# Const-me/Whisper

Hardware: AMD Instinct MI355X
Metric: audio-seconds/sec (real-time factor), ggml-medium & large, 30s chunks @1/2/4/8 GPU (higher is better)
Workload: dtype f16

## Files before the change

### whisper_amd/binding.py

```python
from __future__ import annotations

import ctypes as C
import os
from typing import Optional, Sequence

import numpy as np

from . import ggml_format as gf

_HERE = os.path.dirname(os.path.abspath(__file__))
LIB_PATH = os.path.join(_HERE, "lib", "libwhisper_hip.so")

WH_FLAG_PARITY_PV = 1
WH_FLAG_NO_GRAPH = 2
WH_FLAG_DEBUG_CAPTURE = 4
WH_FLAG_PARITY_EXACT = 8
TUNE_GEMM_8WAVE = 16
TUNE_GEMM_4WAVE = 4
TUNE_GEMM_FAST_EPI = 1
TUNE_GEMV_ROWS4, TUNE_GEMM_BIG, TUNE_GEMV_SMALLREG, TUNE_GEMM_GL, TUNE_LN_SEPARATE_BIGM, TUNE_ATTN_XCD = 2, 8, 32, 64, 128, 256
TUNE_ATTN_DEC_G, TUNE_FUSE_CROSS_Q, TUNE_GEMM_GROUP_M, TUNE_FUSE_SELF_BLOCK, TUNE_GEMV_LN_BLOCK, TUNE_GEMV_K8 = 512, 1024, 2048, 4096, 8192, 16384
TUNE_SPLIT_STREAMS, TUNE_ATTN_ENC_F, TUNE_GEMM_WIDE_EPI, TUNE_GEMM_FRAGPF, TUNE_ATTN_ENC_2SWEEP = 32768, 65536, 131072, 262144, 524288
TUNE_GEMV_ALLROWS, TUNE_GEMV_ROWGROUPS, TUNE_SELF_MFMA, TUNE_MEL_MFMA = 1048576, 2097152, 4194304, 8388608
TUNE_DECODE_SMALL, TUNE_DECODE_PREFETCH, TUNE_ATTN_DEC_NT, TUNE_ENC_SERIAL = 16777216, 33554432, 67108864, 134217728
# ... 95 lines not shown
        L.wh_context_destroy.restype = None
        L.wh_context_set_flags.argtypes = [vp, C.c_uint32, i32]
        L.wh_context_set_audio_ctx.argtypes = [vp, i32]
        L.wh_context_memory.argtypes = [vp, C.POINTER(i64)]
        L.wh_context_synchronize.argtypes = [vp]
        L.wh_buffer_upload_async.argtypes = [vp, vp, vp, i64]
        L.wh_mel_spectrogram.argtypes = [vp, vp, i64, vp, C.POINTER(i64)]
        L.wh_encode.argtypes = [vp, vp, i32, i64, i64, vp]
        L.wh_encode_windows.argtypes = [vp, vp, i32]
        L.wh_decode.argtypes = [vp, vp, i32, i32, i32, vp, vp]
        L.wh_sample_best.argtypes = [vp, i32, i32, i32, C.POINTER(TokenDataC)]
        L.wh_beam_candidates.argtypes = [vp, i32, i32, i32, i32, C.POINTER(TokenDataC)]
        L.wh_reorder_self_cache.argtypes = [vp, i32, vp, i32]
        L.wh_debug_read.argtypes = [vp, C.c_char_p, i32, i32, vp, i64]
        L.wh_decode_greedy.argtypes = [vp, i32, vp, i32, i32, i32, i32, C.POINTER(TokenDataC)]
        L.wh_decode_window_start.argtypes = [vp, i32, vp, i32, i32, i32, i32]
        L.wh_decode_window_finish.argtypes = [vp, C.POINTER(TokenDataC)]
        L.wh_decode_window_start_ragged.argtypes = [vp, i32, vp, vp, i32, i32, i32, i32]
        L.wh_decode_window_ready.argtypes = [vp, i32, i32]
        L.wh_decode_window_continue.argtypes = [vp, i32]
        L.wh_decode_window_fetch.argtypes = [vp, i32, i32, C.POINTER(TokenDataC)]
        L.wh_mel_spectrogram_window.argtypes = [vp, vp, i64, i64, i64, i64, i32, vp]
        L.wh_mel_spectrogram_batch.argtypes = [vp, vp, i64, i64, i32, vp, i64]
        L.wh_debug_probe.argtypes = [vp, i32, i32, i32, i32, i32, i32, C.POINTER(C.c_float)]
        L.wh_profile_enable.argtypes = [vp, i32]
        L.wh_profile_read.argtypes = [vp, C.POINTER(ProfileEntryC), i32, C.POINTER(i32)]
        L.wh_op_mul_mat.argtypes = [vp, vp, vp, vp, vp, vp, i32, i32, i32]
        L.wh_op_mul_mat_gelu.argtypes = [vp, vp, vp, vp, vp, i32, i32, i32]
        L.wh_op_layer_norm.argtypes = [vp, vp, vp, vp, vp, i32, i32]
        L.wh_op_flash_attention.argtypes = [vp, vp, vp, vp, vp, i32, i32, i32]
        L.wh_op_soft_max.argtypes = [vp, vp, i32, i32]
        L.wh_op_decoder_attention.argtypes = [vp, vp, vp, vp, vp, i32, i32, i32, i32, i32, i32, i32, i32, i32]
        L.wh_op_decoder_cross_attention.argtypes = [vp, vp, vp, vp, vp, vp, C.c_float, vp, vp, vp, i32, i32, i32, i32, i32]
        L.wh_op_vocab_soft_max.argtypes = [vp, vp, vp, i32, i32]
        L.wh_op_sample_best.argtypes = [vp, vp, i32, i32, i32, i32, i32, i32, i32, i32, vp]
        L.wh_op_beam_candidates.argtypes = [vp, vp, i32, i32, i32, i32, i32, i32, i32, i32, i32, vp]
        L.wh_op_reorder_self_cache.argtypes = [vp, vp, vp, vp, vp, vp, vp, i32, i32, i32, i32, i32, i32]
        L.wh_lang_detect.argtypes = [vp, i32, vp, vp]
        L.wh_model_lang_count.argtypes = [vp]
        L.wh_op_lang_probs.argtypes = [vp, vp, i32, i32, i32, i32, vp, vp]
        _lib = L
    return _lib


def check(rc: int):
    if rc != 0:
        raise WhisperHipError("libwhisper_hip rc=%d: %s" % (rc, lib().wh_last_error().decode(errors="replace")))


def set_option(name: str, value: int):
    check(lib().wh_debug_set_option(name.encode(), int(value)))


OPTION_DEFAULTS = {"dec_tile": 0, "dec_depth": 0, "dec_wide_rows": 1, "dec_deep_rows": 0, "vocab_decrows": 0, "enc_chunk": 128, "self_fuse_max_rows": 32, "self_nq": 0, "self_wave_min_rows": 32, "enc_exp": 5, "exact_enc_layers": -1, "exact_alt_order": 0, "gemm_mf16": 1, "dec_lds": 1, "dec_lds_ks": 2, "dec_split": 1, "cross_mfma": 1, "vocab_lds": 1, "beam_regs": 1, "reorder_group": 1, "gemm_big_min_rows": 8192}


def get_option(name: str) -> int:
    v = C.c_int(0)
    check(lib().wh_debug_get_option(name.encode(), C.byref(v)))
    return v.value


def get_option_default(name: str) -> int:
    return OPTION_DEFAULTS[name]


def device_count() -> int:
    return lib().wh_device_count()


def device_info(device: int = 0):
    name = C.create_string_buffer(256)
    mem = C.c_uint64()
    cus = C.c_int()
    check(lib().wh_device_info(device, name, 256, C.byref(mem), C.byref(cus)))
    return dict(name=name.value.decode(), total_mem=mem.value, compute_units=cus.value)


def _hp_c(hp: gf.HParams) -> HParamsC:
    return HParamsC(*hp.as_list())


def arena_bytes(hp: gf.HParams) -> int:
    n = lib().wh_model_arena_bytes(C.byref(_hp_c(hp)))
    if n < 0:
        check(-1)
    return int(n)


class HipModel:

    def __init__(self, hp: gf.HParams, arena_ptr: int = 0, already_filled: bool = False, keepalive=None):
        self.hp = hp
        self.handle = C.c_void_p()
        self._keepalive = keepalive
        check(lib().wh_model_create(C.byref(_hp_c(hp)), C.c_void_p(arena_ptr) if arena_ptr else None, int(already_filled),
                                    C.byref(self.handle)))

    @classmethod
    def from_ggml(cls, model: gf.GgmlModel, arena_ptr: int = 0, keepalive=None) -> "HipModel":
        m = cls(model.hparams, arena_ptr, False, keepalive)
        L = lib()
        filt = np.ascontiguousarray(model.filters, np.float32)
        check(L.wh_model_set_filters(m.handle, filt.shape[0], filt.shape[1], filt.ctypes.data_as(C.c_void_p)))
        for name, a in model.tensors.items():
            a = np.ascontiguousarray(a)
            ne = (C.c_int32 * a.ndim)(*reversed(a.shape))
# ... 327 lines not shown
```

### whisper_amd/build.py

```python
from __future__ import annotations

import os
import subprocess
import sys
import time
from concurrent.futures import ThreadPoolExecutor

HERE = os.path.dirname(os.path.abspath(__file__))
ROOT = os.path.dirname(HERE)
CSRC = os.path.join(HERE, "csrc")
HOST = os.path.join(HERE, "host")
LIB_DIR = os.path.join(HERE, "lib")
HIP_LIB = os.path.join(LIB_DIR, "libwhisper_hip.so")
HOST_LIB = os.path.join(LIB_DIR, "libWhisper.so")
CLI_BIN = os.path.join(LIB_DIR, "whisper-main")

RUNTIME_SOURCES = ["options.hip", "model.hip", "comm.hip", "context.hip", "encode.hip", "exact_graphs.hip", "decode.hip", "beam.hip", "ops_debug.hip"]
HIP_SOURCES = ["gemm.hip", "decode1.hip", "attn_enc.hip", "attn_dec.hip", "elementwise.hip", "mel.hip", "exact.hip"] + RUNTIME_SOURCES
EXTRA_FLAGS = {"exact.hip": ["-ffp-contract=off"]}
HIPCC = os.environ.get("HIPCC", "/opt/rocm/bin/hipcc")
ARCH = "gfx950"


def _newer(target: str, deps) -> bool:
    if not os.path.exists(target):
        return True
    t = os.path.getmtime(target)
    return any(os.path.getmtime(d) > t for d in deps)


def _run(cmd):
    print("+", " ".join(cmd), flush=True)
    r = subprocess.run(cmd, stdout=subprocess.PIPE, stderr=subprocess.STDOUT, text=True)
    if r.returncode != 0:
        sys.stderr.write(r.stdout)
        raise RuntimeError("build step failed: " + " ".join(cmd))
    return r.stdout


def build_hip(force: bool = False) -> str:
    os.makedirs(LIB_DIR, exist_ok=True)
    objs = []
    headers = [os.path.join(CSRC, h) for h in ("common.h", "kernels.h", "epilogue.h", "exact_ops.h")] + [os.path.join(ROOT, "include", "whisper_hip.h")]
    obj_dir = os.path.join(LIB_DIR, "obj")
    os.makedirs(obj_dir, exist_ok=True)
    stale = []
    for s in HIP_SOURCES:
        src = os.path.join(CSRC, s)
        obj = os.path.join(obj_dir, s.replace(".hip", ".o"))
        deps = [src] + headers + ([os.path.join(CSRC, "runtime.h")] if s in RUNTIME_SOURCES else [])
        if force or _newer(obj, deps):
            probes = ["-DWH_PROBES"] if os.environ.get("WH_PROBES", "") not in ("", "0") else []
            stale.append([HIPCC, "--offload-arch=" + ARCH, "-O3", "-std=c++17", "-fPIC", "-fvisibility=hidden", "-Wno-unused-result"] + probes + EXTRA_FLAGS.get(s, []) +
                         ["-I" + os.path.join(ROOT, "include"), "-c", src, "-o", obj])
        objs.append(obj)
    with ThreadPoolExecutor(max_workers=max(1, min(16, int(os.environ.get("MAX_JOBS", "0") or 0) or os.cpu_count() or 1))) as pool:
        list(pool.map(_run, stale))
    if force or _newer(HIP_LIB, objs):
        _run([HIPCC, "--offload-arch=" + ARCH, "-shared", "-fPIC", "-o", HIP_LIB] + objs + ["-ldl"])
    return HIP_LIB


def build_host(force: bool = False):
    if not os.path.isdir(HOST):
        return None
    srcs = sorted(os.path.join(HOST, f) for f in os.listdir(HOST) if f.endswith(".cpp"))
    if not srcs:
        return None
    hdrs = [os.path.join(HOST, f) for f in os.listdir(HOST) if f.endswith(".h")]
    hdrs += [os.path.join(ROOT, "include", f) for f in os.listdir(os.path.join(ROOT, "include"))]
    if force or _newer(HOST_LIB, srcs + hdrs + [HIP_LIB]):
        _run(["g++", "-std=c++17", "-O2", "-fPIC", "-shared", "-fvisibility=hidden", "-I" + os.path.join(ROOT, "include"), "-I" + HOST,
# ... 77 lines not shown
```

### whisper_amd/csrc/attn_enc.hip

```cpp
#include "kernels.h"
#include <type_traits>

namespace wh
{
	namespace
	{
		constexpr int AQ = 64;
		constexpr int AWAVES = 8;
		constexpr int QSTRIDE = 72;
		constexpr int OSTRIDE = 65;
		constexpr int ATT_LDS_BYTES = AQ * QSTRIDE * 2 + 2 * AWAVES * AQ * 4 + AWAVES * AQ * 8 + 4 * AQ * OSTRIDE * 4;

		template<int KT>
		__global__ void __launch_bounds__( 512, 2 ) attentionEnc( const f16* __restrict__ q, const f16* __restrict__ k,
			const f16* __restrict__ vT, f16* __restrict__ out, int heads, int T, int Tpad, int nQ, int xcdRemap )
		{
			extern __shared__ __attribute__( ( aligned( 16 ) ) ) unsigned char smem[];
			f16* const ldsQ = (f16*)smem;
			float* const redMax = (float*)( smem + AQ * QSTRIDE * 2 );
			float* const redInv = redMax + AWAVES * AQ;
			double* const redSum = (double*)( redInv + AWAVES * AQ );
			float* const obuf = (float*)( redSum + AWAVES * AQ );

			const int tid = threadIdx.x;
// ... 624 lines not shown
							P[ r >> 3 ][ ( r & 7 ) + 1 ] = ldsTab[ mag[ 1 ] ];
						}
						else
						{
							typedef float f2 __attribute__( ( ext_vector_type( 2 ) ) );
							constexpr float L2E = 1.44269504088896340736f;
							const h2 hp = __builtin_convertvector( f2{ S[ r ] - mx, S[ r + 1 ] - mx }, h2 );
							const f2 e = { __builtin_amdgcn_exp2f( __builtin_fmaf( (float)hp[ 0 ], L2E, 0.0f ) ), __builtin_amdgcn_exp2f( __builtin_fmaf( (float)hp[ 1 ], L2E, 0.0f ) ) };
							const h2 eh = __builtin_convertvector( e, h2 );
							P[ r >> 3 ][ r & 7 ] = eh[ 0 ];
							P[ r >> 3 ][ ( r & 7 ) + 1 ] = eh[ 1 ];
						}
					}
					sum += (double)sumP( P );
	#pragma unroll
					for( int half = 0; half < 2; half++ )
					{
						const int kb = st * 2 + half;
	#pragma unroll
						for( int ddt = 0; ddt < 2; ddt++ )
						{
							const f16x8 vf = *(const f16x8*)( vt + ( ( kb * 2 + ddt ) * 64 + lane ) * 8 );
							O[ ddt ] = __builtin_amdgcn_mfma_f32_32x32x16_f16( vf, P[ half ], O[ ddt ], 0, 0, 0 );
						}
					}
				}
			}
			sum += __shfl_xor( sum, 32, 64 );
			const float invSum = (float)( 1.0 / sum );
	#pragma unroll
			for( int a = 0; a < 2; a++ )
	#pragma unroll
				for( int r = 0; r < 16; r++ ) O[ a ][ r ] *= invSum;
			if( qRow < T )
			{
				const int b = bh / heads, h = bh - b * heads;
				f16* const o = out + ( (long long)b * T + qRow ) * ( heads * HEAD_DIM ) + h * HEAD_DIM;
	#pragma unroll
				for( int ddt = 0; ddt < 2; ddt++ )
	#pragma unroll
					for( int g4 = 0; g4 < 4; g4++ )
					{
						f16x4 pk;
	#pragma unroll
						for( int e = 0; e < 4; e++ ) pk[ e ] = (f16)O[ ddt ][ 4 * g4 + e ];
						*(f16x4*)( o + ddt * 32 + 8 * g4 + 4 * hi ) = pk;
					}
			}
		}

		constexpr int W_NBUF = 4;
		constexpr int W_LDS_BYTES = 2 * W_NBUF * F_TILE * 2;
		constexpr float W_LAZY = 4.0f;
		template<int NG, bool ONLINE, bool NOARG = false>
		__global__ void __launch_bounds__( 1024 / NG, NG == 1 ? 4 : 2 ) attentionEncW( const f16* __restrict__ q, const f16* __restrict__ k,
			const f16* __restrict__ vT, f16* __restrict__ out, int heads, int T, int Tpad, int nQ, int xcdRemap )
		{
			extern __shared__ __attribute__( ( aligned( 16 ) ) ) unsigned char smemW[];
			f16* const ldsK = (f16*)smemW;
			f16* const ldsV = ldsK + W_NBUF * F_TILE;
			typedef __attribute__( ( address_space( 3 ) ) ) void* LdsPtr;
			typedef const __attribute__( ( address_space( 1 ) ) ) void* GlobalPtr;
			typedef _Float16 h2 __attribute__( ( ext_vector_type( 2 ) ) );
			typedef float f2 __attribute__( ( ext_vector_type( 2 ) ) );
			constexpr float L2E = 1.44269504088896340736f;

			const int tid = threadIdx.x;
			const int lane = tid & 63;
			const int wave = tid >> 6;
			const int hi = lane >> 5;
			const int c = lane & 31;
			int bh, qb;
			{
				const int L = blockIdx.x;
				if( xcdRemap )
				{
					const int kIdx = L >> 3;
					bh = ( L & 7 ) + 8 * ( kIdx / nQ );
					qb = kIdx % nQ;
				}
				else
				{
					bh = L / nQ;
					qb = L - bh * nQ;
				}
			}
			const f16* const Q = q + (long long)bh * T * HEAD_DIM;
			const f16* const K = k + (long long)bh * T * HEAD_DIM;
			const f16* const VT = vT + (long long)bh * HEAD_DIM * Tpad;
			const int nTiles = ( T + FK - 1 ) / FK;
			int qRow[ NG ];
			f16x8 qf[ NG ][ 4 ];
	#pragma unroll
			for( int g = 0; g < NG; g++ )
			{
				qRow[ g ] = qb * TQ + ( wave * NG + g ) * 32 + c;
				const int qr = qRow[ g ] < T ? qRow[ g ] : T - 1;
	#pragma unroll
				for( int kk = 0; kk < 4; kk++ )
				{
					qf[ g ][ kk ] = *(const f16x8*)( Q + (long long)qr * HEAD_DIM + kk * 16 + hi * 8 );
	#pragma unroll
					for( int j = 0; j < 8; j++ ) qf[ g ][ kk ][ j ] = qf[ g ][ kk ][ j ] * (f16)0.125f;
				}
			}
			auto issueK = [ & ]( int t, int buf )
			{
	#pragma unroll
				for( int i = 0; i < NG; i++ )
				{
					const int row = ( wave * NG + i ) * 8 + ( lane >> 3 );
					const int cl = ( lane & 7 ) ^ ( ( row >> 1 ) & 7 );
					int key = t * FK + row;
					key = key < T ? key : T - 1;
					__builtin_amdgcn_global_load_lds( (GlobalPtr)( K + (long long)key * HEAD_DIM + cl * 8 ),
						(LdsPtr)( ldsK + buf * F_TILE + ( wave * NG + i ) * 512 ), 16, 0, 0 );
				}
			};
			auto issueV = [ & ]( int t, int buf )
			{
	#pragma unroll
				for( int i = 0; i < NG; i++ )
					__builtin_amdgcn_global_load_lds( (GlobalPtr)( VT + (long long)t * F_TILE + ( wave * NG + i ) * 512 + lane * 8 ),
						(LdsPtr)( ldsV + buf * F_TILE + ( wave * NG + i ) * 512 ), 16, 0, 0 );
			};
			auto waitTile = [ & ]( int t, auto per )
			{
				constexpr int P = decltype( per )::value;
				const int younger = min( W_NBUF - 2, nTiles - 1 - t );
				if( younger >= 2 )
				{
					if constexpr( P == 2 ) asm volatile( "s_waitcnt vmcnt(4)" ::: "memory" );
					else asm volatile( "s_waitcnt vmcnt(8)" ::: "memory" );
				}
				else if( younger == 1 )
				{
					if constexpr( P == 2 ) asm volatile( "s_waitcnt vmcnt(2)" ::: "memory" );
					else asm volatile( "s_waitcnt vmcnt(4)" ::: "memory" );
				}
				else asm volatile( "s_waitcnt vmcnt(0)" ::: "memory" );
			};
			static_assert( W_NBUF == 4 && NG == 2, "waitTile counts two younger tiles of 2 or 4 load instructions" );
			const f32x16 zero16 = { 0, 0, 0, 0, 0, 0, 0, 0, 0, 0, 0, 0, 0, 0, 0, 0 };
			auto scores = [ & ]( const f16* kt, int st, int t, auto last, f32x16 ( &S )[ NG ] )
			{
				const int row = st * 32 + c;
				const int sw = ( row >> 1 ) & 7;
	#pragma unroll
				for( int kk = 0; kk < 4; kk++ )
				{
					const f16x8 kf = *(const f16x8*)( kt + row * HEAD_DIM + ( ( ( kk * 2 + hi ) ^ sw ) << 3 ) );
	#pragma unroll
					for( int g = 0; g < NG; g++ ) S[ g ] = __builtin_amdgcn_mfma_f32_32x32x16_f16( kf, qf[ g ][ kk ], kk == 0 ? zero16 : S[ g ], 0, 0, 0 );
				}
				if constexpr( decltype( last )::value )
				{
					const int limit = T - ( t * FK + st * 32 + 4 * hi );
	#pragma unroll
					for( int r = 0; r < 16; r++ )
					{
						const bool in = ( r & 3 ) + 8 * ( r >> 2 ) < limit;
	#pragma unroll
						for( int g = 0; g < NG; g++ ) S[ g ][ r ] = in ? S[ g ][ r ] : -3.0e38f;
					}
				}
			};
			auto sumP = [ & ]( const f16x8 ( &P )[ 2 ] ) -> float
			{
				const h2 ones = { (f16)1.0f, (f16)1.0f };
				float part = 0.0f;
	#pragma unroll
				for( int h = 0; h < 2; h++ )
	#pragma unroll
					for( int j = 0; j < 8; j += 2 )
						part = __builtin_amdgcn_fdot2( h2{ P[ h ][ j ], P[ h ][ j + 1 ] }, ones, part, false );
				return part;
			};
			auto expTile = [ & ]( const f32x16& S, float mref, f16x8 ( &P )[ 2 ] )
			{
	#pragma unroll
				for( int r = 0; r < 16; r += 2 )
				{
					f2 e;
					if constexpr( NOARG )
					{
						const float mL = mref * L2E;
						e = f2{ __builtin_amdgcn_exp2f( __builtin_fmaf( S[ r ], L2E, -mL ) ), __builtin_amdgcn_exp2f( __builtin_fmaf( S[ r + 1 ], L2E, -mL ) ) };
					}
					else
					{
						const h2 hd = __builtin_convertvector( f2{ S[ r ] - mref, S[ r + 1 ] - mref }, h2 );
						e = f2{ __builtin_amdgcn_exp2f( __builtin_fmaf( (float)hd[ 0 ], L2E, 0.0f ) ), __builtin_amdgcn_exp2f( __builtin_fmaf( (float)hd[ 1 ], L2E, 0.0f ) ) };
					}
					const h2 eh = __builtin_convertvector( e, h2 );
					P[ r >> 3 ][ r & 7 ] = eh[ 0 ];
					P[ r >> 3 ][ ( r & 7 ) + 1 ] = eh[ 1 ];
				}
			};

			float mx[ NG ];
	#pragma unroll
			for( int g = 0; g < NG; g++ ) mx[ g ] = -INFINITY;
			if constexpr( !ONLINE )
			{
	#pragma unroll
				for( int i = 0; i < W_NBUF - 1; i++ )
					if( i < nTiles ) issueK( i, i );
				for( int t = 0; t < nTiles; t++ )
				{
					waitTile( t, std::integral_constant<int, NG>{} );
					__syncthreads();
					if( t + W_NBUF - 1 < nTiles ) issueK( t + W_NBUF - 1, ( t + W_NBUF - 1 ) % W_NBUF );
					const f16* const kt = ldsK + ( t % W_NBUF ) * F_TILE;
					auto body = [ & ]( auto last )
					{
	#pragma unroll
						for( int st = 0; st < 4; st++ )
						{
							f32x16 S[ NG ];
							scores( kt, st, t, last, S );
	#pragma unroll
							for( int g = 0; g < NG; g++ )
	#pragma unroll
								for( int r = 0; r < 16; r++ ) mx[ g ] = fmaxf( mx[ g ], S[ g ][ r ] );
						}
					};
					if( t == nTiles - 1 ) body( std::true_type{} ); else body( std::false_type{} );
				}
	#pragma unroll
				for( int g = 0; g < NG; g++ ) mx[ g ] = fmaxf( mx[ g ], __shfl_xor( mx[ g ], 32, 64 ) );
				__syncthreads();
			}

			double sum[ NG ];
			float sumF[ NG ];
			f32x16 O[ NG ][ 2 ];
	#pragma unroll
			for( int g = 0; g < NG; g++ )
			{
				sum[ g ] = 0.0;
				sumF[ g ] = 0.0f;
	#pragma unroll
				for( int a = 0; a < 2; a++ )
	#pragma unroll
					for( int r = 0; r < 16; r++ ) O[ g ][ a ][ r ] = 0.0f;
			}
	#pragma unroll
			for( int i = 0; i < W_NBUF - 1; i++ )
				if( i < nTiles ) { issueK( i, i ); issueV( i, i ); }
			for( int t = 0; t < nTiles; t++ )
			{
				waitTile( t, std::integral_constant<int, 2 * NG>{} );
				__syncthreads();
				if( t + W_NBUF - 1 < nTiles )
				{
					issueK( t + W_NBUF - 1, ( t + W_NBUF - 1 ) % W_NBUF );
					issueV( t + W_NBUF - 1, ( t + W_NBUF - 1 ) % W_NBUF );
				}
				const f16* const kt = ldsK + ( t % W_NBUF ) * F_TILE;
				const f16* const vt = ldsV + ( t % W_NBUF ) * F_TILE;
				auto body = [ & ]( auto last )
				{
	#pragma unroll
					for( int st = 0; st < 4; st++ )
					{
						f32x16 S[ NG ];
						scores( kt, st, t, last, S );
						if constexpr( ONLINE )
						{
							float tm[ NG ];
							bool raise = false;
	#pragma unroll
							for( int g = 0; g < NG; g++ )
							{
								tm[ g ] = S[ g ][ 0 ];
	#pragma unroll
								for( int r = 1; r < 16; r++ ) tm[ g ] = fmaxf( tm[ g ], S[ g ][ r ] );
								tm[ g ] = fmaxf( tm[ g ], __shfl_xor( tm[ g ], 32, 64 ) );
								raise = raise || tm[ g ] > mx[ g ] + W_LAZY;
							}
							if( __any( raise ) )
							{
	#pragma unroll
								for( int g = 0; g < NG; g++ )
								{
									const float mNew = tm[ g ] > mx[ g ] + W_LAZY ? tm[ g ] : mx[ g ];
									const float f = __builtin_amdgcn_exp2f( ( mx[ g ] - mNew ) * L2E );
									mx[ g ] = mNew;
									sumF[ g ] *= f;
	#pragma unroll
									for( int a = 0; a < 2; a++ )
	#pragma unroll
										for( int r = 0; r < 16; r++ ) O[ g ][ a ][ r ] *= f;
								}
							}
						}
						f16x8 P[ NG ][ 2 ];
	#pragma unroll
						for( int g = 0; g < NG; g++ )
						{
							expTile( S[ g ], mx[ g ], P[ g ] );
							if constexpr( ONLINE ) sumF[ g ] += sumP( P[ g ] );
							else sum[ g ] += (double)sumP( P[ g ] );
						}
	#pragma unroll
						for( int half = 0; half < 2; half++ )
						{
							const int kb = st * 2 + half;
	#pragma unroll
							for( int ddt = 0; ddt < 2; ddt++ )
							{
								const f16x8 vf = *(const f16x8*)( vt + ( ( kb * 2 + ddt ) * 64 + lane ) * 8 );
	#pragma unroll
								for( int g = 0; g < NG; g++ ) O[ g ][ ddt ] = __builtin_amdgcn_mfma_f32_32x32x16_f16( vf, P[ g ][ half ], O[ g ][ ddt ], 0, 0, 0 );
							}
						}
					}
				};
				if( t == nTiles - 1 ) body( std::true_type{} ); else body( std::false_type{} );
			}
	#pragma unroll
			for( int g = 0; g < NG; g++ )
			{
				if constexpr( ONLINE ) sum[ g ] = (double)sumF[ g ];
				sum[ g ] += __shfl_xor( sum[ g ], 32, 64 );
				const float invSum = (float)( 1.0 / sum[ g ] );
				if( qRow[ g ] < T )
				{
					const int b = bh / heads, h = bh - b * heads;
					f16* const o = out + ( (long long)b * T + qRow[ g ] ) * ( heads * HEAD_DIM ) + h * HEAD_DIM;
	#pragma unroll
					for( int ddt = 0; ddt < 2; ddt++ )
	#pragma unroll
						for( int g4 = 0; g4 < 4; g4++ )
						{
							f16x4 pk;
	#pragma unroll
							for( int e = 0; e < 4; e++ ) pk[ e ] = (f16)( O[ g ][ ddt ][ 4 * g4 + e ] * invSum );
							*(f16x4*)( o + ddt * 32 + 8 * g4 + 4 * hi ) = pk;
						}
				}
			}
		}

		template<int NG, bool ONLINE, bool NOARG = false>
		int launchEncWideT( const f16* q, const f16* k, const f16* vT, f16* out, int batch, int heads, int T, int Tpad, hipStream_t stream )
		{
			static PerDeviceOnce once;
			if( const int onceDev = once.needed(); onceDev >= 0 )
			{
				WH_HIP( hipFuncSetAttribute( (const void*)attentionEncW<NG, ONLINE, NOARG>, hipFuncAttributeMaxDynamicSharedMemorySize, W_LDS_BYTES ) );
				once.mark( onceDev );
			}
			const int nQ = ( T + TQ - 1 ) / TQ, BH = batch * heads;
			const int xcdRemap = ( BH % 8 ) == 0 && ( g_tuning & TUNE_ATTN_XCD ) ? 1 : 0;
			hipLaunchKernelGGL( ( attentionEncW<NG, ONLINE, NOARG> ), dim3( nQ * BH ), dim3( 1024 / NG ), W_LDS_BYTES, stream, q, k, vT, out, heads, T, Tpad, nQ, xcdRemap );
			WH_HIP( hipGetLastError() );
			return 0;
		}
		int launchEncWide( const f16* q, const f16* k, const f16* vT, f16* out, int batch, int heads, int T, int Tpad, int mode, hipStream_t stream )
		{
			if( mode == 5 ) return launchEncWideT<2, true, true>( q, k, vT, out, batch, heads, T, Tpad, stream );
			if( mode == 3 ) return launchEncWideT<2, true>( q, k, vT, out, batch, heads, T, Tpad, stream );
			return launchEncWideT<2, false>( q, k, vT, out, batch, heads, T, Tpad, stream );
		}

		int launchEncTable( const f16* q, const f16* k, const f16* vT, f16* out, int batch, int heads, int T, int Tpad, const f16* expTab, hipStream_t stream )
		{
			static PerDeviceOnce once;
			if( const int onceDev = once.needed(); onceDev >= 0 )
			{
				WH_HIP( hipFuncSetAttribute( (const void*)attentionEncT<0>, hipFuncAttributeMaxDynamicSharedMemorySize, T_LDS_BYTES ) );
				WH_HIP( hipFuncSetAttribute( (const void*)attentionEncT<1>, hipFuncAttributeMaxDynamicSharedMemorySize, T_LDS_BYTES - T_TABLE_HALFS * 2 ) );
				once.mark( onceDev );
			}
			const int nQ = ( T + TQ - 1 ) / TQ, BH = batch * heads;
			const int xcdRemap = ( BH % 8 ) == 0 && ( g_tuning & TUNE_ATTN_XCD ) ? 1 : 0;
			if( g_opt.encExp == 2 || g_opt.encExp == 3 || g_opt.encExp == 5 ) return launchEncWide( q, k, vT, out, batch, heads, T, Tpad, g_opt.encExp, stream );
			if( g_opt.encExp == 1 )
				hipLaunchKernelGGL( attentionEncT<1>, dim3( nQ * BH ), dim3( 1024 ), T_LDS_BYTES - T_TABLE_HALFS * 2, stream, q, k, vT, out, expTab, heads, T, Tpad, nQ, xcdRemap );
			else
			hipLaunchKernelGGL( attentionEncT<0>, dim3( nQ * BH ), dim3( 1024 ), T_LDS_BYTES, stream, q, k, vT, out, expTab, heads, T, Tpad, nQ, xcdRemap );
			WH_HIP( hipGetLastError() );
			return 0;
		}

		int launchEncF( const f16* q, const f16* k, const f16* vT, f16* out, int batch, int heads, int T, int Tpad, bool exactP, hipStream_t stream )
		{
			static PerDeviceOnce once;
			if( const int onceDev = once.needed(); onceDev >= 0 )
			{
				WH_HIP( hipFuncSetAttribute( (const void*)attentionEncF<false>, hipFuncAttributeMaxDynamicSharedMemorySize, F_LDS_BYTES ) );
				WH_HIP( hipFuncSetAttribute( (const void*)attentionEncF<true>, hipFuncAttributeMaxDynamicSharedMemorySize, F_LDS_BYTES ) );
				once.mark( onceDev );
			}
			const int nQ = ( T + FQ - 1 ) / FQ, BH = batch * heads;
			const int xcdRemap = ( BH % 8 ) == 0 && ( g_tuning & TUNE_ATTN_XCD ) ? 1 : 0;
			const bool two = !exactP && ( g_tuning & TUNE_ATTN_ENC_2SWEEP );
			if( two )
				hipLaunchKernelGGL( attentionEncF<true>, dim3( nQ * BH ), dim3( 512 ), F_LDS_BYTES, stream, q, k, vT, out, heads, T, Tpad, nQ, xcdRemap );
			else
				hipLaunchKernelGGL( attentionEncF<false>, dim3( nQ * BH ), dim3( 512 ), F_LDS_BYTES, stream, q, k, vT, out, heads, T, Tpad, nQ, xcdRemap );
			WH_HIP( hipGetLastError() );
			return 0;
		}

		template<int KT>
		int launchEncT( const f16* q, const f16* k, const f16* vT, f16* out, int batch, int heads, int T, int Tpad, hipStream_t stream )
		{
			static PerDeviceOnce once;
			if( const int onceDev = once.needed(); onceDev >= 0 )
			{
				WH_HIP( hipFuncSetAttribute( (const void*)attentionEnc<KT>, hipFuncAttributeMaxDynamicSharedMemorySize, ATT_LDS_BYTES ) );
				once.mark( onceDev );
			}
			const int nQ = ( T + AQ - 1 ) / AQ, BH = batch * heads;
			const int xcdRemap = ( BH % 8 ) == 0 && ( g_tuning & TUNE_ATTN_XCD ) ? 1 : 0;
			hipLaunchKernelGGL( attentionEnc<KT>, dim3( nQ * BH ), dim3( 512 ), ATT_LDS_BYTES, stream, q, k, vT, out, heads, T, Tpad, nQ, xcdRemap );
			WH_HIP( hipGetLastError() );
			return 0;
		}
	}

	int attentionInit() { return 0; }

	int launchAttentionEnc( const f16* q, const f16* k, const f16* vT, f16* out, int batch, int heads, int T, int Tpad, bool exactP, const f16* expTab,
		hipStream_t stream )
	{
		if( T <= 0 || T > 1536 || Tpad < ( ( T + 255 ) / 256 ) * 256 || ( Tpad & 7 ) != 0 )
		{
			setError( "attentionEnc: need 0 < T <= 1536 and Tpad >= roundup(T, 256)" );
// ... 18 lines not shown
```

### whisper_amd/csrc/kernels.h

```cpp
#pragma once
#include "common.h"

namespace wh
{
	enum eTuning : unsigned
	{
		TUNE_GEMV_ROWS4 = 2,
		TUNE_GEMM_4WAVE = 4,
		TUNE_GEMM_FAST_EPI = 1,
		TUNE_GEMM_8WAVE = 16,
		TUNE_GEMM_BIG = 8,
		TUNE_GEMV_SMALLREG = 32,
		TUNE_GEMM_GL = 64,
		TUNE_LN_SEPARATE_BIGM = 128,
		TUNE_ATTN_XCD = 256,
		TUNE_ATTN_DEC_G = 512,
		TUNE_FUSE_CROSS_Q = 1024,
		TUNE_FUSE_SELF_BLOCK = 4096,
		TUNE_GEMV_LN_BLOCK = 8192,
		TUNE_GEMV_K8 = 16384,
		TUNE_SPLIT_STREAMS = 32768,
		TUNE_ATTN_ENC_F = 65536,
		TUNE_GEMM_WIDE_EPI = 131072,
		TUNE_GEMM_FRAGPF = 262144,
		TUNE_ATTN_ENC_2SWEEP = 524288,
		TUNE_MEL_MFMA = 8388608,
		TUNE_SELF_MFMA = 4194304,
		TUNE_GEMV_ALLROWS = 1048576,
		TUNE_GEMV_ROWGROUPS = 2097152,
		TUNE_GEMM_GROUP_M = 2048,
		TUNE_ATTN_DEC_NT = 67108864,
		TUNE_DECODE_SMALL = 16777216,
		TUNE_DECODE_PREFETCH = 33554432,
		TUNE_ATTN_ENC_TABLE = 268435456,
		TUNE_ATTN_ENC_TABLE_ANY = 1073741824,
		TUNE_SAMPLE_SPREAD = 2147483648u,
		TUNE_GEMV_MT8 = 536870912,
		TUNE_ENC_SERIAL = 134217728,
		TUNE_DEFAULT = TUNE_GEMM_FAST_EPI | TUNE_GEMM_8WAVE | TUNE_GEMV_ROWS4 | TUNE_GEMV_SMALLREG | TUNE_GEMM_BIG | TUNE_GEMM_GL | TUNE_LN_SEPARATE_BIGM | TUNE_ATTN_XCD | TUNE_ATTN_DEC_G | TUNE_FUSE_CROSS_Q | TUNE_GEMM_GROUP_M | TUNE_FUSE_SELF_BLOCK | TUNE_GEMV_K8 | TUNE_ATTN_ENC_F | TUNE_GEMM_WIDE_EPI | TUNE_GEMM_FRAGPF | TUNE_ATTN_ENC_2SWEEP | TUNE_GEMV_ALLROWS | TUNE_GEMV_ROWGROUPS | TUNE_SELF_MFMA | TUNE_MEL_MFMA | TUNE_DECODE_SMALL | TUNE_ATTN_DEC_NT | TUNE_ATTN_ENC_TABLE
	};
	extern unsigned g_tuning;

	struct Options
	{
		int decTile = 0;
		int decDepth = 0;
		int decWideRows = 1;
		int decDeepRows = 0;
		int vocabDecRows = 0;
		int encChunk = 128;
		int selfFuseMaxRows = 32;
		int selfNq = 0;
		int exactEncLayers = -1;
		int encExp = 5;
		int encAblate = 0;
		int exactAltOrder = 0;
		int decLds = 1;
		int decLdsKs = 2;
		int decSplit = 1;
		int crossMfma = 1;
		int vocabLds = 1;
		int beamRegs = 1;
		int reorderGroup = 1;
		int gemmBigMinRows = 8192;
		int gemmMf16 = 1;
		int selfWaveMinRows = 32;
	};
	extern Options g_opt;

	enum eEpilogue : int
	{
		EPI_F32 = 0,
		EPI_F16_GELU,
		EPI_CONV2,
		EPI_QKV_ENC,
		EPI_CROSS_KV,
		EPI_QKV_DEC,
		EPI_Q_DEC,
	};

	struct GemmArgs
	{
		const f16* A;
		const f16* W;
		int M, N, K;
		int lda, Mb;
		long long aBatchStride;
		int epi;
		const float* bias;
		const float* res;
		float* out32;
		f16* out16;
		int ldc;
		long long cBatchStride;
		const float* pe;
		float scale;
		f16* q;
		f16* k;
		f16* v;
		int T, Tpad, H, B;
		int nTok, nPast, textCtx;
		const int* nPastDev;
		const float* lnX;
		const float* lnW;
		const float* lnB;
		int wideEpi;
		int groupM;
// ... 201 lines not shown
```

Baseline: 10390.

## Add one-wave-per-SIMD software-pipelined encoder attention kernel and make it default

Adds an ONE variant of the wide encoder attention kernel that runs 256 threads (4 waves) per block. It hand-schedules each 32-key subtile so the next subtile's QK MFMAs, the exp/convert/row-sum work and the K fragment loads for the following subtile interleave with the PV MFMAs, separated by sched_barrier fences. K/V DMA pieces are issued in staggered slots inside the loop, with explicit vmcnt waits. The kernel is compiled with the mfma-vgpr-form LLVM flag and becomes the default encoder path (enc_exp=6). It trades occupancy (one block per CU) and a lot of code complexity for better overlap of MFMA, transcendental and memory work, with risk around waitcnt accounting and register pressure.

```diff
diff --git a/whisper_amd/binding.py b/whisper_amd/binding.py
--- a/whisper_amd/binding.py
+++ b/whisper_amd/binding.py
@@ -171,7 +171,7 @@
     check(lib().wh_debug_set_option(name.encode(), int(value)))
 
 
-OPTION_DEFAULTS = {"dec_tile": 0, "dec_depth": 0, "dec_wide_rows": 1, "dec_deep_rows": 0, "vocab_decrows": 0, "enc_chunk": 128, "self_fuse_max_rows": 32, "self_nq": 0, "self_wave_min_rows": 32, "enc_exp": 5, "exact_enc_layers": -1, "exact_alt_order": 0, "gemm_mf16": 1, "dec_lds": 1, "dec_lds_ks": 2, "dec_split": 1, "cross_mfma": 1, "vocab_lds": 1, "beam_regs": 1, "reorder_group": 1, "gemm_big_min_rows": 8192}
+OPTION_DEFAULTS = {"dec_tile": 0, "dec_depth": 0, "dec_wide_rows": 1, "dec_deep_rows": 0, "vocab_decrows": 0, "enc_chunk": 128, "self_fuse_max_rows": 32, "self_nq": 0, "self_wave_min_rows": 32, "enc_exp": 6, "exact_enc_layers": -1, "exact_alt_order": 0, "gemm_mf16": 1, "dec_lds": 1, "dec_lds_ks": 2, "dec_split": 1, "cross_mfma": 1, "vocab_lds": 1, "beam_regs": 1, "reorder_group": 1, "gemm_big_min_rows": 8192}
 
 
 def get_option(name: str) -> int:
diff --git a/whisper_amd/build.py b/whisper_amd/build.py
--- a/whisper_amd/build.py
+++ b/whisper_amd/build.py
@@ -17,7 +17,7 @@
 
 RUNTIME_SOURCES = ["options.hip", "model.hip", "comm.hip", "context.hip", "encode.hip", "exact_graphs.hip", "decode.hip", "beam.hip", "ops_debug.hip"]
 HIP_SOURCES = ["gemm.hip", "decode1.hip", "attn_enc.hip", "attn_dec.hip", "elementwise.hip", "mel.hip", "exact.hip"] + RUNTIME_SOURCES
-EXTRA_FLAGS = {"exact.hip": ["-ffp-contract=off"]}
+EXTRA_FLAGS = {"exact.hip": ["-ffp-contract=off"], "attn_enc.hip": ["-mllvm", "-amdgpu-mfma-vgpr-form"]}
 HIPCC = os.environ.get("HIPCC", "/opt/rocm/bin/hipcc")
 ARCH = "gfx950"
 
diff --git a/whisper_amd/csrc/attn_enc.hip b/whisper_amd/csrc/attn_enc.hip
--- a/whisper_amd/csrc/attn_enc.hip
+++ b/whisper_amd/csrc/attn_enc.hip
@@ -700,10 +700,13 @@
 		constexpr int W_NBUF = 4;
 		constexpr int W_LDS_BYTES = 2 * W_NBUF * F_TILE * 2;
 		constexpr float W_LAZY = 4.0f;
-		template<int NG, bool ONLINE, bool NOARG = false>
-		__global__ void __launch_bounds__( 1024 / NG, NG == 1 ? 4 : 2 ) attentionEncW( const f16* __restrict__ q, const f16* __restrict__ k,
+		template<int NG, bool ONLINE, bool NOARG = false, bool ONE = false>
+		__global__ void __launch_bounds__( ONE ? 256 : 1024 / NG, ONE ? 1 : NG == 1 ? 4 : 2 ) attentionEncW( const f16* __restrict__ q, const f16* __restrict__ k,
 			const f16* __restrict__ vT, f16* __restrict__ out, int heads, int T, int Tpad, int nQ, int xcdRemap )
 		{
+			constexpr int NW = ONE ? 4 : 16 / NG;
+			constexpr int PCS = 16 / NW;
+			constexpr int WQ = NW * NG * 32;
 			extern __shared__ __attribute__( ( aligned( 16 ) ) ) unsigned char smemW[];
 			f16* const ldsK = (f16*)smemW;
 			f16* const ldsV = ldsK + W_NBUF * F_TILE;
@@ -742,7 +745,7 @@
 	#pragma unroll
 			for( int g = 0; g < NG; g++ )
 			{
-				qRow[ g ] = qb * TQ + ( wave * NG + g ) * 32 + c;
+				qRow[ g ] = qb * WQ + ( wave * NG + g ) * 32 + c;
 				const int qr = qRow[ g ] < T ? qRow[ g ] : T - 1;
 	#pragma unroll
 				for( int kk = 0; kk < 4; kk++ )
@@ -755,40 +758,44 @@
 			auto issueK = [ & ]( int t, int buf )
 			{
 	#pragma unroll
-				for( int i = 0; i < NG; i++ )
-				{
-					const int row = ( wave * NG + i ) * 8 + ( lane >> 3 );
+				for( int i = 0; i < PCS; i++ )
+				{
+					const int row = ( wave * PCS + i ) * 8 + ( lane >> 3 );
 					const int cl = ( lane & 7 ) ^ ( ( row >> 1 ) & 7 );
 					int key = t * FK + row;
 					key = key < T ? key : T - 1;
 					__builtin_amdgcn_global_load_lds( (GlobalPtr)( K + (long long)key * HEAD_DIM + cl * 8 ),
-						(LdsPtr)( ldsK + buf * F_TILE + ( wave * NG + i ) * 512 ), 16, 0, 0 );
+						(LdsPtr)( ldsK + buf * F_TILE + ( wave * PCS + i ) * 512 ), 16, 0, 0 );
 				}
 			};
 			auto issueV = [ & ]( int t, int buf )
 			{
 	#pragma unroll
-				for( int i = 0; i < NG; i++ )
-					__builtin_amdgcn_global_load_lds( (GlobalPtr)( VT + (long long)t * F_TILE + ( wave * NG + i ) * 512 + lane * 8 ),
-						(LdsPtr)( ldsV + buf * F_TILE + ( wave * NG + i ) * 512 ), 16, 0, 0 );
-			};
-			auto waitTile = [ & ]( int t, auto per )
+				for( int i = 0; i < PCS; i++ )
+					__builtin_amdgcn_global_load_lds( (GlobalPtr)( VT + (long long)t * F_TILE + ( wave * PCS + i ) * 512 + lane * 8 ),
+						(LdsPtr)( ldsV + buf * F_TILE + ( wave * PCS + i ) * 512 ), 16, 0, 0 );
+			};
+			auto waitTile = [ & ]( int t, auto per, auto ahead )
 			{
 				constexpr int P = decltype( per )::value;
-				const int younger = min( W_NBUF - 2, nTiles - 1 - t );
+				static_assert( P == 2 || P == 4 || P == 8, "waitTile's immediates" );
+				const int younger = min( (int)decltype( ahead )::value, nTiles - 1 - t );
 				if( younger >= 2 )
 				{
 					if constexpr( P == 2 ) asm volatile( "s_waitcnt vmcnt(4)" ::: "memory" );
+					else if constexpr( P == 4 ) asm volatile( "s_waitcnt vmcnt(8)" ::: "memory" );
+					else asm volatile( "s_waitcnt vmcnt(16)" ::: "memory" );
+				}
+				else if( younger == 1 )
+				{
+					if constexpr( P == 2 ) asm volatile( "s_waitcnt vmcnt(2)" ::: "memory" );
+					else if constexpr( P == 4 ) asm volatile( "s_waitcnt vmcnt(4)" ::: "memory" );
 					else asm volatile( "s_waitcnt vmcnt(8)" ::: "memory" );
 				}
-				else if( younger == 1 )
-				{
-					if constexpr( P == 2 ) asm volatile( "s_waitcnt vmcnt(2)" ::: "memory" );
-					else asm volatile( "s_waitcnt vmcnt(4)" ::: "memory" );
-				}
 				else asm volatile( "s_waitcnt vmcnt(0)" ::: "memory" );
 			};
-			static_assert( W_NBUF == 4 && NG == 2, "waitTile counts two younger tiles of 2 or 4 load instructions" );
+			static_assert( W_NBUF == 4 && NW * PCS == 16 && ( !ONE || ONLINE ), "waitTile counts at most two younger tiles; the one-wave-per-SIMD form is the one-sweep kernel" );
+			constexpr std::integral_constant<int, W_NBUF - 2> ringAhead{};
 			const f32x16 zero16 = { 0, 0, 0, 0, 0, 0, 0, 0, 0, 0, 0, 0, 0, 0, 0, 0 };
 			auto scores = [ & ]( const f16* kt, int st, int t, auto last, f32x16 ( &S )[ NG ] )
 			{
@@ -856,7 +863,7 @@
 					if( i < nTiles ) issueK( i, i );
 				for( int t = 0; t < nTiles; t++ )
 				{
-					waitTile( t, std::integral_constant<int, NG>{} );
+					waitTile( t, std::integral_constant<int, PCS>{}, ringAhead );
 					__syncthreads();
 					if( t + W_NBUF - 1 < nTiles ) issueK( t + W_NBUF - 1, ( t + W_NBUF - 1 ) % W_NBUF );
 					const f16* const kt = ldsK + ( t % W_NBUF ) * F_TILE;
@@ -895,10 +902,232 @@
 			}
 	#pragma unroll
 			for( int i = 0; i < W_NBUF - 1; i++ )
-				if( i < nTiles ) { issueK( i, i ); issueV( i, i ); }
+				if( i < nTiles )
+				{
+					issueK( i, i );
+					if( !ONE || i < W_NBUF - 2 ) issueV( i, i );
+				}
+			if constexpr( ONE )
+			{
+				static_assert( NG == 2, "the gaps below are laid out for two query groups per wave" );
+				const h2 ones = { (f16)1.0f, (f16)1.0f };
+				auto gap = [] { __builtin_amdgcn_sched_barrier( 0 ); };
+				auto loadKf = [ & ]( const f16* kt, int st, int kk ) -> f16x8
+				{
+					const int row = st * 32 + c;
+					return *(const f16x8*)( kt + row * HEAD_DIM + ( ( ( kk * 2 + hi ) ^ ( ( row >> 1 ) & 7 ) ) << 3 ) );
+				};
+				auto maskHalf = [ & ]( f32x16& S, int t, int st, int half )
+				{
+					const int limit = T - ( t * FK + st * 32 + 4 * hi );
+	#pragma unroll
+					for( int r = half * 8; r < half * 8 + 8; r++ ) S[ r ] = ( r & 3 ) + 8 * ( r >> 2 ) < limit ? S[ r ] : -3.0e38f;
+				};
+				auto issuePiece = [ & ]( int tl, int idx )
+				{
+					const int piece = wave * PCS + ( idx & 3 ), buf = tl % W_NBUF;
+					if( idx < 4 )
+					{
+						const int row = piece * 8 + ( lane >> 3 );
+						const int cl = ( lane & 7 ) ^ ( ( row >> 1 ) & 7 );
+						int key = tl * FK + row;
+						key = key < T ? key : T - 1;
+						__builtin_amdgcn_global_load_lds( (GlobalPtr)( K + (long long)key * HEAD_DIM + cl * 8 ), (LdsPtr)( ldsK + buf * F_TILE + piece * 512 ), 16, 0, 0 );
+					}
+					else
+						__builtin_amdgcn_global_load_lds( (GlobalPtr)( VT + (long long)tl * F_TILE + piece * 512 + lane * 8 ), (LdsPtr)( ldsV + buf * F_TILE + piece * 512 ), 16, 0, 0 );
+				};
+				auto subTile = [ & ]( const f16* vt, int st, auto pre, auto mask, int tNext, int stNext, const f16x8 ( &kfN )[ 4 ], auto ld, const f16* ktLd, int stLd,
+					f16x8 ( &kfL )[ 4 ], f32x16 ( &Sc )[ NG ], f32x16 ( &Sn )[ NG ], float ( &tm )[ NG ], auto dma, int tDma, int pc )
+				{
+					constexpr bool PRE = decltype( pre )::value, MASK = decltype( mask )::value, LD = decltype( ld )::value, DMA = decltype( dma )::value;
+					bool raise = false;
+	#pragma unroll
+					for( int g = 0; g < NG; g++ ) raise = raise || tm[ g ] > mx[ g ] + W_LAZY;
+					if( __any( raise ) )
+					{
+	#pragma unroll
+						for( int g = 0; g < NG; g++ )
+						{
+							const float mNew = tm[ g ] > mx[ g ] + W_LAZY ? tm[ g ] : mx[ g ];
+							const float f = __builtin_amdgcn_exp2f( ( mx[ g ] - mNew ) * L2E );
+							mx[ g ] = mNew;
+							sumF[ g ] *= f;
+	#pragma unroll
+							for( int a = 0; a < 2; a++ )
+	#pragma unroll
+								for( int r = 0; r < 16; r++ ) O[ g ][ a ][ r ] *= f;
+						}
+					}
+					float mL[ NG ], part[ NG ], tmN[ NG ], tmO[ NG ];
+	#pragma unroll
+					for( int g = 0; g < NG; g++ )
+					{
+						mL[ g ] = mx[ g ] * L2E;
+						part[ g ] = 0.0f;
+					}
+					f16x8 vf[ 2 ][ 2 ], P[ NG ][ 2 ];
+					f2 ef[ 16 ];
+					auto E = [ & ]( int p )
+					{
+						const int g = ( p >> 2 ) & 1, r = ( p >> 3 ) * 8 + 2 * ( p & 3 );
+						if constexpr( NOARG ) ef[ p ] = f2{ __builtin_amdgcn_exp2f( __builtin_fmaf( Sc[ g ][ r ], L2E, -mL[ g ] ) ), __builtin_amdgcn_exp2f( __builtin_fmaf( Sc[ g ][ r + 1 ], L2E, -mL[ g ] ) ) };
+						else
+						{
+							const h2 hd = __builtin_convertvector( f2{ Sc[ g ][ r ] - mx[ g ], Sc[ g ][ r + 1 ] - mx[ g ] }, h2 );
+							ef[ p ] = f2{ __builtin_amdgcn_exp2f( __builtin_fmaf( (float)hd[ 0 ], L2E, 0.0f ) ), __builtin_amdgcn_exp2f( __builtin_fmaf( (float)hd[ 1 ], L2E, 0.0f ) ) };
+						}
+					};
+					auto Cv = [ & ]( int p )
+					{
+						const h2 eh = __builtin_convertvector( ef[ p ], h2 );
+						P[ ( p >> 2 ) & 1 ][ p >> 3 ][ 2 * ( p & 3 ) ] = eh[ 0 ];
+						P[ ( p >> 2 ) & 1 ][ p >> 3 ][ 2 * ( p & 3 ) + 1 ] = eh[ 1 ];
+					};
+					auto Dt = [ & ]( int p )
+					{
+						const int g = ( p >> 2 ) & 1, j = 2 * ( p & 3 );
+						part[ g ] = __builtin_amdgcn_fdot2( h2{ P[ g ][ p >> 3 ][ j ], P[ g ][ p >> 3 ][ j + 1 ] }, ones, part[ g ], false );
+					};
+					gap();
+	#pragma unroll
+					for( int i = 0; i < 8; i++ )
+					{
+						if constexpr( PRE ) Sn[ i & 1 ] = __builtin_amdgcn_mfma_f32_32x32x16_f16( kfN[ i >> 1 ], qf[ i & 1 ][ i >> 1 ], i < 2 ? zero16 : Sn[ i & 1 ], 0, 0, 0 );
+						if( i < 4 ) vf[ i >> 1 ][ i & 1 ] = *(const f16x8*)( vt + ( ( ( st * 2 + ( i >> 1 ) ) * 2 + ( i & 1 ) ) * 64 + lane ) * 8 );
+						E( i );
+						if( i >= 1 ) Cv( i - 1 );
+						if( i >= 2 ) Dt( i - 2 );
+						gap();
+					}
+	#pragma unroll
+					for( int i = 0; i < 4; i++ )
+					{
+						O[ i & 1 ][ i >> 1 ] = __builtin_amdgcn_mfma_f32_32x32x16_f16( vf[ 0 ][ i >> 1 ], P[ i & 1 ][ 0 ], O[ i & 1 ][ i >> 1 ], 0, 0, 0 );
+						if constexpr( LD ) kfL[ i ] = loadKf( ktLd, stLd, i );
+						E( 8 + 2 * i );
+						E( 9 + 2 * i );
+						if( i == 0 )
+						{
+							Cv( 7 );
+							Dt( 6 );
+						}
+						else
+						{
+							Cv( 6 + 2 * i );
+							Cv( 7 + 2 * i );
+							Dt( 4 + 2 * i + ( i == 1 ? 1 : 0 ) );
+							if( i >= 2 ) Dt( 5 + 2 * i );
+						}
+						if( i == 3 ) sumF[ 0 ] += part[ 0 ];
+						gap();
+					}
+					auto tailGap = [ & ]( auto ic )
+					{
+						constexpr int i = decltype( ic )::value;
+						O[ i & 1 ][ i >> 1 ] = __builtin_amdgcn_mfma_f32_32x32x16_f16( vf[ 1 ][ i >> 1 ], P[ i & 1 ][ 1 ], O[ i & 1 ][ i >> 1 ], 0, 0, 0 );
+						if( i == 0 )
+						{
+							Cv( 14 );
+							Cv( 15 );
+							Dt( 12 );
+							Dt( 13 );
+						}
+						if( i == 1 )
+						{
+							Dt( 14 );
+							Dt( 15 );
+							sumF[ 1 ] += part[ 1 ];
+						}
+						if constexpr( PRE )
+							if( i < NG )
+							{
+								if constexpr( MASK )
+								{
+									maskHalf( Sn[ i ], tNext, stNext, 0 );
+									maskHalf( Sn[ i ], tNext, stNext, 1 );
+								}
+								tmN[ i ] = Sn[ i ][ 0 ];
+	#pragma unroll
+								for( int r = 1; r < 16; r++ ) tmN[ i ] = fmaxf( tmN[ i ], Sn[ i ][ r ] );
+								tmO[ i ] = __shfl_xor( tmN[ i ], 32, 64 );
+							}
+						if constexpr( DMA && i >= 2 ) issuePiece( tDma, pc + i - 2 );
+						gap();
+					};
+					tailGap( std::integral_constant<int, 0>{} );
+					tailGap( std::integral_constant<int, 1>{} );
+					tailGap( std::integral_constant<int, 2>{} );
+					tailGap( std::integral_constant<int, 3>{} );
+					if constexpr( PRE )
+					{
+	#pragma unroll
+						for( int g = 0; g < NG; g++ ) tm[ g ] = fmaxf( tmN[ g ], tmO[ g ] );
+					}
+				};
+
+				f32x16 S[ 2 ][ NG ];
+				f16x8 kfA[ 4 ], kfB[ 4 ];
+				float tm[ NG ];
+				constexpr std::true_type yes{};
+				constexpr std::false_type no{};
+				if( nTiles >= 3 ) asm volatile( "s_waitcnt vmcnt(12)" ::: "memory" );
+				else if( nTiles == 2 ) asm volatile( "s_waitcnt vmcnt(8)" ::: "memory" );
+				else asm volatile( "s_waitcnt vmcnt(0)" ::: "memory" );
+				__syncthreads();
+	#pragma unroll
+				for( int kk = 0; kk < 4; kk++ ) kfA[ kk ] = loadKf( ldsK, 0, kk );
+	#pragma unroll
+				for( int kk = 0; kk < 4; kk++ ) kfB[ kk ] = loadKf( ldsK, 1, kk );
+	#pragma unroll
+				for( int kk = 0; kk < 4; kk++ )
+	#pragma unroll
+					for( int g = 0; g < NG; g++ ) S[ 0 ][ g ] = __builtin_amdgcn_mfma_f32_32x32x16_f16( kfA[ kk ], qf[ g ][ kk ], kk == 0 ? zero16 : S[ 0 ][ g ], 0, 0, 0 );
+	#pragma unroll
+				for( int g = 0; g < NG; g++ )
+				{
+					if( nTiles == 1 )
+					{
+						maskHalf( S[ 0 ][ g ], 0, 0, 0 );
+						maskHalf( S[ 0 ][ g ], 0, 0, 1 );
+					}
+					float m = S[ 0 ][ g ][ 0 ];
+	#pragma unroll
+					for( int r = 1; r < 16; r++ ) m = fmaxf( m, S[ 0 ][ g ][ r ] );
+					tm[ g ] = fmaxf( m, __shfl_xor( m, 32, 64 ) );
+				}
+				auto tile = [ & ]( int t, auto nextIsLast, auto dmaV, auto dmaK )
+				{
+					const f16* const kt = ldsK + ( t % W_NBUF ) * F_TILE;
+					const f16* const vt = ldsV + ( t % W_NBUF ) * F_TILE;
+					const f16* const ktN = ldsK + ( ( t + 1 ) % W_NBUF ) * F_TILE;
+					subTile( vt, 0, yes, no, t, 1, kfB, yes, kt, 2, kfA, S[ 0 ], S[ 1 ], tm, dmaV, t + 2, 4 );
+					subTile( vt, 1, yes, no, t, 2, kfA, yes, kt, 3, kfB, S[ 1 ], S[ 0 ], tm, dmaV, t + 2, 6 );
+					if constexpr( decltype( dmaV )::value ) asm volatile( "s_waitcnt vmcnt(8)" : "+v"( sumF[ 0 ] ), "+v"( sumF[ 1 ] ) : : "memory" );
+					else asm volatile( "s_waitcnt vmcnt(0)" : "+v"( sumF[ 0 ] ), "+v"( sumF[ 1 ] ) : : "memory" );
+					static_assert( 2 * PCS == 8, "a tile is 8 load instructions per wave" );
+					__syncthreads();
+					subTile( vt, 2, yes, no, t, 3, kfB, yes, ktN, 0, kfA, S[ 0 ], S[ 1 ], tm, dmaK, t + W_NBUF - 1, 0 );
+					subTile( vt, 3, yes, nextIsLast, t + 1, 0, kfA, yes, ktN, 1, kfB, S[ 1 ], S[ 0 ], tm, dmaK, t + W_NBUF - 1, 2 );
+				};
+				for( int t = 0; t < nTiles - 3; t++ ) tile( t, no, yes, yes );
+				if( nTiles >= 3 ) tile( nTiles - 3, no, yes, no );
+				if( nTiles >= 2 ) tile( nTiles - 2, yes, no, no );
+				{
+					const int t = nTiles - 1;
+					const f16* const kt = ldsK + ( t % W_NBUF ) * F_TILE;
+					const f16* const vt = ldsV + ( t % W_NBUF ) * F_TILE;
+					const int nSub = ( T - t * FK + 31 ) >> 5;
+					subTile( vt, 0, yes, yes, t, 1, kfB, yes, kt, 2, kfA, S[ 0 ], S[ 1 ], tm, no, 0, 0 );
+					if( nSub > 1 ) subTile( vt, 1, yes, yes, t, 2, kfA, yes, kt, 3, kfB, S[ 1 ], S[ 0 ], tm, no, 0, 0 );
+					if( nSub > 2 ) subTile( vt, 2, yes, yes, t, 3, kfB, no, kt, 3, kfA, S[ 0 ], S[ 1 ], tm, no, 0, 0 );
+					if( nSub > 3 ) subTile( vt, 3, no, no, t, 3, kfA, no, kt, 3, kfB, S[ 1 ], S[ 0 ], tm, no, 0, 0 );
+				}
+			}
+			else
 			for( int t = 0; t < nTiles; t++ )
 			{
-				waitTile( t, std::integral_constant<int, 2 * NG>{} );
+				waitTile( t, std::integral_constant<int, 2 * PCS>{}, ringAhead );
 				__syncthreads();
 				if( t + W_NBUF - 1 < nTiles )
 				{
@@ -991,23 +1220,25 @@
 			}
 		}
 
-		template<int NG, bool ONLINE, bool NOARG = false>
+		template<int NG, bool ONLINE, bool NOARG = false, bool ONE = false>
 		int launchEncWideT( const f16* q, const f16* k, const f16* vT, f16* out, int batch, int heads, int T, int Tpad, hipStream_t stream )
 		{
 			static PerDeviceOnce once;
 			if( const int onceDev = once.needed(); onceDev >= 0 )
 			{
-				WH_HIP( hipFuncSetAttribute( (const void*)attentionEncW<NG, ONLINE, NOARG>, hipFuncAttributeMaxDynamicSharedMemorySize, W_LDS_BYTES ) );
+				WH_HIP( hipFuncSetAttribute( (const void*)attentionEncW<NG, ONLINE, NOARG, ONE>, hipFuncAttributeMaxDynamicSharedMemorySize, W_LDS_BYTES ) );
 				once.mark( onceDev );
 			}
-			const int nQ = ( T + TQ - 1 ) / TQ, BH = batch * heads;
+			constexpr int threads = ONE ? 256 : 1024 / NG, rows = ( threads / 64 ) * NG * 32;
+			const int nQ = ( T + rows - 1 ) / rows, BH = batch * heads;
 			const int xcdRemap = ( BH % 8 ) == 0 && ( g_tuning & TUNE_ATTN_XCD ) ? 1 : 0;
-			hipLaunchKernelGGL( ( attentionEncW<NG, ONLINE, NOARG> ), dim3( nQ * BH ), dim3( 1024 / NG ), W_LDS_BYTES, stream, q, k, vT, out, heads, T, Tpad, nQ, xcdRemap );
+			hipLaunchKernelGGL( ( attentionEncW<NG, ONLINE, NOARG, ONE> ), dim3( nQ * BH ), dim3( threads ), W_LDS_BYTES, stream, q, k, vT, out, heads, T, Tpad, nQ, xcdRemap );
 			WH_HIP( hipGetLastError() );
 			return 0;
 		}
 		int launchEncWide( const f16* q, const f16* k, const f16* vT, f16* out, int batch, int heads, int T, int Tpad, int mode, hipStream_t stream )
 		{
+			if( mode == 6 ) return launchEncWideT<2, true, true, true>( q, k, vT, out, batch, heads, T, Tpad, stream );
 			if( mode == 5 ) return launchEncWideT<2, true, true>( q, k, vT, out, batch, heads, T, Tpad, stream );
 			if( mode == 3 ) return launchEncWideT<2, true>( q, k, vT, out, batch, heads, T, Tpad, stream );
 			return launchEncWideT<2, false>( q, k, vT, out, batch, heads, T, Tpad, stream );
@@ -1024,7 +1255,7 @@
 			}
 			const int nQ = ( T + TQ - 1 ) / TQ, BH = batch * heads;
 			const int xcdRemap = ( BH % 8 ) == 0 && ( g_tuning & TUNE_ATTN_XCD ) ? 1 : 0;
-			if( g_opt.encExp == 2 || g_opt.encExp == 3 || g_opt.encExp == 5 ) return launchEncWide( q, k, vT, out, batch, heads, T, Tpad, g_opt.encExp, stream );
+			if( g_opt.encExp == 2 || g_opt.encExp == 3 || g_opt.encExp >= 5 ) return launchEncWide( q, k, vT, out, batch, heads, T, Tpad, g_opt.encExp, stream );
 			if( g_opt.encExp == 1 )
 				hipLaunchKernelGGL( attentionEncT<1>, dim3( nQ * BH ), dim3( 1024 ), T_LDS_BYTES - T_TABLE_HALFS * 2, stream, q, k, vT, out, expTab, heads, T, Tpad, nQ, xcdRemap );
 			else
diff --git a/whisper_amd/csrc/kernels.h b/whisper_amd/csrc/kernels.h
--- a/whisper_amd/csrc/kernels.h
+++ b/whisper_amd/csrc/kernels.h
@@ -52,7 +52,7 @@
 		int selfFuseMaxRows = 32;
 		int selfNq = 0;
 		int exactEncLayers = -1;
-		int encExp = 5;
+		int encExp = 6;
 		int encAblate = 0;
 		int exactAltOrder = 0;
 		int decLds = 1;
```

New measurement: 10340. About the same (-0.5%).
